# akloetgen/PARA-suite

Measured on AMD Instinct MI355X. Metric: aligned reads/sec (10Mx50bp PAR-CLIP vs hg19-size genome) on MI355X; SAM bit-exact vs own CPU restatement (parity unpinned), higher is better.
Workload: dtype u64

## Files before the change

para-suite_amd/capi.py:

```python
import ctypes as C
import os

import numpy as np

_HERE = os.path.dirname(os.path.abspath(__file__))
SO_PATH = os.environ.get("PARASUITE_LIB") or os.path.join(_HERE, "libparasuite_hip.so")


class IndexInfo(C.Structure):
    _fields_ = [("seq_len", C.c_uint64), ("l_pac", C.c_uint64), ("primary", C.c_uint64), ("L2", C.c_uint64 * 5),
                ("n_blocks", C.c_uint64), ("n_sa", C.c_uint64), ("device_bytes", C.c_uint64),
                ("n_contigs", C.c_int32), ("n_holes", C.c_int32), ("sa_rounds", C.c_int32), ("sa_intv", C.c_int32),
                ("build_ms", C.c_double), ("jump_levels", C.c_int32), ("pad_", C.c_int32)]


class Timing(C.Structure):
    _fields_ = [("ms_width", C.c_double), ("ms_backtrack", C.c_double), ("ms_compact", C.c_double),
                ("ms_select", C.c_double), ("ms_sa2pos", C.c_double), ("ms_refine", C.c_double),
                ("ms_host_post", C.c_double), ("ms_total", C.c_double), ("n_width_launches", C.c_int32),
                ("n_backtrack_launches", C.c_int32), ("n_overflow_tier1", C.c_int64), ("n_overflow_tier2", C.c_int64),
                ("ms_classify", C.c_double), ("ms_rows", C.c_double), ("ms_sel_hard", C.c_double), ("ms_sel_easy", C.c_double),
                ("bt_begin_ms", C.c_double), ("bt_end_ms", C.c_double)]


# ... 192 lines not shown
        k = np.ascontiguousarray(keys, dtype=np.uint8)
        out = np.empty(k.size, dtype=np.int32)
        _chk(lib().ps_ctx_order_sort(self.h, k.ctypes.data, k.size, out.ctypes.data))
        return out

    def export_blob(self, which, dev_ptr, nbytes):
        _chk(lib().ps_ctx_export_blob(self.h, which, dev_ptr, nbytes))

    def bwt_syms_chunked(self, chunk_blocks=1 << 20):
        info = self.info()
        blk = self.fetch(0).view("<u4").reshape(-1, 16)
        out = np.empty(blk.shape[0] * 192, dtype=np.uint8)
        sh = np.arange(32, dtype=np.uint32)[None, None, :]
        for a in range(0, blk.shape[0], chunk_blocks):
            lo = (blk[a:a + chunk_blocks, 4:10, None] >> sh) & 1
            hi = (blk[a:a + chunk_blocks, 10:16, None] >> sh) & 1
            out[a * 192:(a + lo.shape[0]) * 192] = (lo | (hi << 1)).astype(np.uint8).reshape(-1)
        return out[:info.seq_len]

    def bwt_syms(self):
        blk = self.fetch(0).view("<u4").reshape(-1, 16)
        return self.bwt_syms_chunked(), blk[:, :4]

    RI_WORDS = 20

    def read_iters(self):
        n = lib().ps_ctx_read_iters(self.h, None, 0)
        out = np.zeros(n, dtype=np.uint32)
        lib().ps_ctx_read_iters(self.h, out.ctypes.data, n)
        return out

    def batch_from_fastq(self, path):
        return Batch(lib().ps_batch_from_fastq(self.h, path.encode()), self)

    def batch_from_codes(self, codes):
        c = np.ascontiguousarray(codes, dtype=np.uint8)
        return Batch(lib().ps_batch_from_codes(self.h, c.shape[0], c.shape[1], c.ctypes.data), self)


class Batch:
    def __init__(self, handle, ctx):
        if not handle:
            raise PsError(lib().ps_last_error().decode())
        self.h = handle
        self.ctx = ctx

    def free(self):
# ... 228 lines not shown
```

para-suite_amd/csrc/ps_effort.hip:

```cpp
#include <hip/hip_runtime.h>
#include "ps_core.h"
#include <stdexcept>
#include "ps_kernels.h"
#include "ps_budget.h"

namespace ps {

struct EChain {
    bwtint k, l;
    uint32_t cost_lo, cost_hi;
    int piece;
    int n_rs;
    int cl_n, cl_last;
    uint32_t cl_lo, cl_hi;
};
__device__ __forceinline__ void echain_restart(const EffortArgs &a, EChain &c, bool lo_half)
{
    c.k = 0; c.l = a.ix.seq_len; c.piece = 0; c.cl_n = 0; ++c.n_rs;
    if (lo_half) c.cost_lo += (uint32_t)a.c_restart; else c.cost_hi += (uint32_t)a.c_restart;
}
__device__ __forceinline__ void echain_step(const EffortArgs &a, EChain &c, int sym, uint32_t cw, int pos, bool lo_half, LaneStats &st)
{
    uint32_t ck[4], cl[4];
    occ_pair4(a.ix.blocks, a.ix.primary, c.k, c.l, ck, cl, st);
    if (sym < 4) {
        const uint32_t ok = sel4(ck, sym), ol = sel4(cl, sym);
        if (ok < ol) { const bwtint b = L2_of(a.ix, sym); c.k = b + ok + 1; c.l = b + ol; ++c.piece; return; }
    }
    int best = -1; uint32_t best_cost = 0xffu;
    if (c.l - c.k < (bwtint)a.w_pin) {
#pragma unroll
        for (int t = 0; t < 4; ++t) {
            const uint32_t ct = (cw >> (8 * t)) & 0xffu;
            if (t != sym && ck[t] < cl[t] && ct < best_cost) { best = t; best_cost = ct; }
        }
    }
    if (best < 0) { echain_restart(a, c, lo_half); return; }
    const int d = pos > c.cl_last ? pos - c.cl_last : c.cl_last - pos;
    if (c.cl_n > 0 && d <= 4) ++c.cl_n; else { c.cl_n = 1; c.cl_lo = c.cost_lo; c.cl_hi = c.cost_hi; }
    c.cl_last = pos;
    if (lo_half) c.cost_lo += best_cost; else c.cost_hi += best_cost;
    if (c.cl_n >= 3) {
        c.k = 0; c.l = a.ix.seq_len; c.piece = 0; c.cl_n = 0; ++c.n_rs;
        return;
    }
    const bwtint b = L2_of(a.ix, best);
    c.k = b + sel4(ck, best) + 1; c.l = b + sel4(cl, best); ++c.piece;
}

__global__ void __launch_bounds__(256, 8) k_effort(EffortArgs a)
{
    const int lane = threadIdx.x & 63;
    const bool is_b = lane >= 32;
    const int wave = (int)((blockIdx.x * blockDim.x + threadIdx.x) >> 6), n_waves = (int)((gridDim.x * blockDim.x) >> 6);
    LaneStats st = {0, 0, 0, 0, 0, 0, 0, 0};
    for (int r = wave * 32 + (lane & 31); r < a.n_reads; r += n_waves * 32) {
        const int len = a.lens ? a.lens[r] : a.len, half = len >> 1;
        EChain C = {0, a.ix.seq_len, 0, 0, 0, 0, 0, 0, 0, 0};
        uint32_t bw = 0, mw = 0;
#pragma unroll 1
        for (int i = 0; i < len; ++i) {
            const int j = is_b ? i : len - 1 - i;
            if (i == 0 || (j & 15) == (is_b ? 0 : 15)) bw = a.bases[(size_t)(j >> 4) * a.n_reads + opaque_lane(r)];
            if (i == 0 || (j & 31) == (is_b ? 0 : 31)) mw = a.nmask[(size_t)(j >> 5) * a.n_reads + opaque_lane(r)];
            const int bs = ((mw >> (j & 31)) & 1u) ? 4 : (int)((bw >> (2 * (j & 15))) & 3u);
            const int sc = bs > 3 ? 4 : 3 - bs;
            const uint32_t cws = cost_word(a.s_pk, sc);
            const uint32_t cw = is_b ? cws : __builtin_bswap32(cws);
            echain_step(a, C, is_b ? sc : bs, cw, j, j < half, st);
        }
        const uint32_t mine = C.cost_lo + C.cost_hi;
        const uint32_t tb = (uint32_t)__shfl((int)mine, lane | 32, 64), ta = mine;
        const int b_rs = __shfl(C.n_rs, lane | 32, 64), a_rs = C.n_rs;
        if (!is_b) {
            const uint32_t e = a_rs == 0 ? (b_rs == 0 && tb < ta ? tb : ta) : (b_rs == 0 ? tb : (ta > tb ? ta : tb));
            a.est[r] = (uint8_t)(e > 255u ? 255u : e);
            if (a.est_ab) a.est_ab[r] = (uint16_t)((ta > 127u ? 127u : ta) | (a_rs ? 0x80u : 0u) | ((tb > 127u ? 127u : tb) << 8) | (b_rs ? 0x8000u : 0u));
        }
    }
}

template <int G>
__global__ void __launch_bounds__(256) k_effort_model(EffortModelArgs a)
{
    const int lane = threadIdx.x & 63, u = lane & (G - 1);
    const int per_wave = 64 / G;
    const long long wave = ((long long)blockIdx.x * blockDim.x + threadIdx.x) >> 6, n_waves = ((long long)gridDim.x * blockDim.x) >> 6;
    for (long long r0 = wave * per_wave + lane / G; r0 < a.n_reads; r0 += n_waves * per_wave) {
        const int r = (int)r0;
        const int len = a.lens ? a.lens[r] : a.len;
        const int own = (a.lens && a.units_by_len) ? (int)a.units_by_len[len] : a.max_units;
        int B = (int)a.est[r] + a.u_tight;
        if (B > own) B = own;
        float w = u == 0 ? 1.f : 0.f;
        float tot = 0.f, phi_rows = a.rows;
        const int depth = len < a.depth ? len : a.depth;
        const int rem = B - u;
        const int m = rem >= 0 ? (int)(((uint32_t)rem * a.inv_c_min) >> 16) : -1;
        const int srem = a.seed_units - u;
        const bool seed_ok = srem > 0 && (int)(((uint32_t)srem * a.inv_c_min) >> 16) >= 1;
// ... 76 lines not shown
```

para-suite_amd/csrc/ps_kernels.h:

```cpp
#pragma once
#include <hip/hip_runtime.h>
#include "ps_types.h"
#include "ps_budget.h"

namespace ps {

static const int PS_MAX_CIGAR = 16;

struct WidthArgs {
    IndexView ix;
    int n_reads, len, seed_len, use_seed;
    const int32_t *lens;
    const uint32_t *bases; const uint32_t *nmask;
    uint32_t *w; uint32_t *cwb; uint32_t *cswb;
    KStats *stats;
};

struct EffortArgs {
    IndexView ix;
    int n_reads, len;
    const int32_t *lens;
    const uint32_t *bases; const uint32_t *nmask;
    uint32_t s_pk[5];
    int c_restart;
    uint32_t w_pin;
    uint8_t *est;
    uint16_t *est_ab;
};

struct EffortModelArgs {
    int n_reads, len;
    const int32_t *lens; const uint8_t *units_by_len;
    const uint32_t *bases; const uint32_t *nmask; const uint32_t *cwb;
    const uint8_t *est;
    uint32_t s_pk[5]; uint32_t inv_c_min;
    int max_units, u_tight, seed_units, use_seed, seed_len;
    int max_gapo, indel_end_skip, u_gapo_ins, u_gapo_del;
    int depth;
    float rows;
    int log_scale;
    uint8_t *key; float *pred;
};

struct RefineItem { int32_t read; bwtint rb; int32_t ref_shift; int32_t strand; };
struct RefineArgs {
    IndexView ix;
    int n_items, len, n_reads;
    const int32_t *lens;
    const uint32_t *bases; const uint32_t *nmask;
    const RefineItem *items;
// ... 24 lines not shown
```

para-suite_amd/csrc/ps_kernels.hip:

```cpp
#include <hip/hip_runtime.h>
#include <algorithm>
#include <cstdlib>
#include <stdexcept>
#include <string>
#include "ps_core.h"
#include "ps_narrow.h"
#include "ps_kernels.h"

namespace ps {

static const int PS_Q_CHUNK = 64;
#ifndef PS_BT_WAVES
#define PS_BT_WAVES 4
#endif

__device__ __forceinline__ unsigned long long wave_sum(unsigned long long v)
{
    for (int o = 32; o > 0; o >>= 1) v += __shfl_xor(v, o, 64);
    return v;
}
__device__ __forceinline__ void flush_stats(KStats *ks, const LaneStats &st)
{
    if (!ks) return;
    unsigned long long v[8] = {st.pairs, st.same, st.nodes, st.pushes, st.pops, st.lf, st.iters, st.exact};
// ... 207 lines not shown
                unsigned int at = atomicAdd(a.big_next, 1u) % n_big;
                for (int tries = 0; tries < 256; ++tries) {
                    if (atomicCAS(a.big_busy + at, 0u, 1u) == 0u) { slot = at; break; }
                    at = at + 1u == n_big ? 0u : at + 1u;
                }
            }
            slot = (unsigned int)__shfl((int)slot, src, 64);
            const unsigned int n_copy = (unsigned int)__shfl((int)nl_bump(L), src, 64);
            const unsigned long long from = (unsigned long long)__shfl((long long)reinterpret_cast<unsigned long long>(m.pool), src, 64);
            if (slot < n_big) {
                const uint4 *sp = reinterpret_cast<const uint4 *>(from);
                uint4 *dp = reinterpret_cast<uint4 *>(a.big_pool + (size_t)slot * h.big_cap * sizeof(Entry16));
                for (unsigned int e = (unsigned int)lane; e < n_copy; e += 64u) dp[e] = sp[e];
                __threadfence();
                if (lane == src) { m.pool = dp; L.ctl = nl_set_mode(L.ctl | NL_BIG, M_EXPAND); }
            } else if (lane == src) L.ctl = nl_set_mode(nl_set_status(L.ctl, RS_OVERFLOW_POOL), M_POP);
        }
        nt_iter<STATS, NB32>(a, h, L, st, m, fetch_r, serve_hit, &clk);
        if (STATS && a.read_iters) {
            const int now = nl_mode(L.ctl);
            if (mode == M_FETCH && now != M_FETCH && now != M_EXIT) {
                iters0 = st.iters - 1u;
                const int len = nl_len(L), sl = h.seed_len();
                a.read_iters[PS_RI_WORDS * (size_t)L.r + 2] = (uint32_t)(m.cw[len - 1] & 0x7f) | ((h.use_seed() && sl > 0 && sl < len ? (uint32_t)(m.csw[sl - 1] & 0x7f) : 0u) << 8) | (a.est_ab ? (uint32_t)a.est_ab[L.r] << 16 : 0u);
                const uint32_t *cw32 = reinterpret_cast<const uint32_t *>(m.cw);
                for (int p = 0; p < 16; ++p) a.read_iters[PS_RI_WORDS * (size_t)L.r + 4 + p] = p < lm_ncw(len) ? cw32[p] : 0u;
            }
            if (mode != M_FETCH && mode != M_EXIT && now == M_FETCH) {
                uint32_t *ri = a.read_iters + PS_RI_WORDS * (size_t)L.r;
                ri[0] = st.iters - iters0; ri[1] = nl_bump(L);
                ri[3] = (uint32_t)nl_best_score(L) | ((uint32_t)nl_max_units(L) << 8) | ((uint32_t)nl_n_aln(L.ctl) << 16);
            }
        }
    }
    if (STATS) {
        if (lane == 0) st.lf = (uint32_t)((wall_clock64() - t_start) >> 4);
#ifdef PS_STAMPS
        st.nodes = lane == 0 ? (uint32_t)(clk.tm[0] >> 6) : 0; st.pushes = lane == 0 ? (uint32_t)(clk.tm[1] >> 6) : 0;
        st.pops = lane == 0 ? (uint32_t)(clk.tm[2] >> 6) : 0; st.exact = lane == 0 ? (uint32_t)(clk.tm[3] >> 6) : 0;
#endif
        flush_stats(a.stats, st);
    } else {
        st.nodes = st.pushes = st.pops = st.iters = st.exact = st.lf = 0;
        flush_stats(a.stats, st);
    }
}

__global__ void __launch_bounds__(256) k_sa2pos(IndexView ix, const bwtint *rows, bwtint *out, int n, KStats *stats)
{
    const int stride = gridDim.x * blockDim.x;
    int item = blockIdx.x * blockDim.x + threadIdx.x;
    LaneStats st = {0, 0, 0, 0, 0, 0, 0, 0};
    bool have = false; bwtint row = 0; uint32_t steps = 0;
    while (true) {
// ... 146 lines not shown
```

para-suite_amd/csrc/ps_narrow.h:

```cpp
#pragma once
#include "ps_core.h"

namespace ps {

PS_HD int nw_i(uint32_t wa) { return (int)(wa & 0xffu); }
PS_HD int nw_ldp(uint32_t wa) { return (int)((wa >> 8) & 0xffu); }
PS_HD int nw_mm(uint32_t wa) { return (int)((wa >> 16) & 0xffu); }
PS_HD int nw_state(uint32_t wa) { return (int)((wa >> 24) & 3u); }
PS_HD int nw_gapo(uint32_t wa) { return (int)((wa >> 26) & 7u); }
PS_HD int nw_gape(uint32_t wa) { return (int)(wa >> 29); }
PS_HD int nw_ins(uint32_t wb) { return (int)(wb & 7u); }
PS_HD int nw_del(uint32_t wb) { return (int)((wb >> 3) & 7u); }
PS_HD uint32_t nw_c(uint32_t wb) { return (wb >> 6) & 7u; }
PS_HD int nw_score(uint32_t wb) { return (int)((wb >> 9) & 0x7fu); }
static const uint32_t NW_KEEP = 0xFCFF0000u;
static const uint32_t NW_C_MASK = 7u << 6;
static const uint32_t NW_ROOT_C = 4u;

PS_HD int nl_mode(uint32_t ctl) { return (int)(ctl & 7u); }
PS_HD uint32_t nl_set_mode(uint32_t ctl, int mode) { return (ctl & ~7u) | (uint32_t)mode; }
static const uint32_t NL_HAVE_CUR = 8u, NL_STATUS = 7u << 4, NL_BIG = 1u << 7;
PS_HD int nl_status(uint32_t ctl) { return (int)((ctl >> 4) & 7u); }
PS_HD uint32_t nl_set_status(uint32_t ctl, int s) { return (ctl & ~NL_STATUS) | ((uint32_t)s << 4); }
PS_HD int nl_n_aln(uint32_t ctl) { return (int)(ctl >> 16); }

struct NLane {
    uint32_t kr, lr, wa, wb;
    uint32_t ctl;
    int r;
    uint32_t lim;
    uint32_t nsb;
    uint32_t n_phantom;
    uint32_t fh;
    uint32_t bm0, bm1;
    uint32_t rn0, rn1;
};
PS_HD int nl_best_score(const NLane &L) { return (int)(L.lim & 0xffu); }
PS_HD int nl_max_units(const NLane &L) { return (int)((L.lim >> 8) & 0xffu); }
PS_HD int nl_len(const NLane &L) { return (int)((L.lim >> 16) & 0xffu); }
PS_HD int nl_n_stack(const NLane &L) { return (int)(L.nsb & 0xffffu); }
PS_HD uint32_t nl_bump(const NLane &L) { return L.nsb >> 16; }
PS_HD uint32_t nl_phantom(const NLane &L) { return L.n_phantom & 0x00FFFFFFu; }
PS_HD int nl_est(const NLane &L) { return (int)(L.n_phantom >> 24); }

// ... 90 lines not shown
        empty = ps[2 * c] >= ps[2 * c + 1];
        kr = ps[2 * c] + 1u; lr = ps[2 * c + 1];
    }
    uint32_t ck[4] = {0, 0, 0, 0}, cl[4] = {0, 0, 0, 0};
    LaneStats st;
    if (!empty) nt_occ<false>(h, c, kr, lr, ck, cl, st);
    uint32_t *out = table + (size_t)(jump_level_off(d) + s) * PS_JUMP_SLOT_WORDS;
    for (int j = 0; j < 4; ++j) { out[2 * j] = ck[j]; out[2 * j + 1] = cl[j]; }
}

PS_HD int nt_seq_at(const BtMem &m, const NLane &L, int j, int len, int max_len)
{
    const int p = len - 1 - j;
    const uint32_t b = (m.rb[p >> 4] >> (2 * (p & 15))) & 3u;
    const uint32_t nw = lm_nmask_in_regs(max_len) ? (p < 32 ? L.rn0 : L.rn1) : m.rn[p >> 5];
    return ((nw >> (p & 31)) & 1u) ? 4 : 3 - (int)b;
}

PS_HD void nt_heads_init(BtMem &m, int n_buckets)
{
    uint32_t *hw = reinterpret_cast<uint32_t *>(m.heads16);
    for (int p = 0; p < (n_buckets + 1) >> 1; ++p) hw[p] = 0xFFFFFFFFu;
}
PS_COLD void nt_restart_without_estimate(const BtArgs &a, NLane &L, BtMem &m)
{
    L.ctl = (L.ctl & NL_BIG) | (uint32_t)M_POP | NL_HAVE_CUR;
    L.kr = 0; L.lr = (uint32_t)a.ix.seq_len; L.wa = (uint32_t)nl_len(L); L.wb = NW_ROOT_C << 6;
    L.lim = (L.lim & 0x00FFFF00u) | 0xffu;
    L.nsb = 0; L.bm0 = L.bm1 = 0; L.fh = 0xffffu; L.n_phantom = 0xFF000000u;
    nt_heads_init(m, a.md.n_buckets);
}
PS_HD void nt_finish_read(const BtArgs &a, NLane &L)
{
    a.n_aln[L.r] = nl_n_aln(L.ctl);
    a.status[L.r] = (uint8_t)nl_status(L.ctl);
    L.ctl = nl_set_mode(L.ctl, M_FETCH);
}

PS_COLD void nt_hit(const BtArgs &a, NLane &L, BtMem &m)
{
    const Model &md = a.md;
    const uint32_t c = nw_c(L.wb);
    if (a.ix.jump && c != NW_ROOT_C) {
        const int d = nt_depth(nl_len(L), L.wa, L.wb);
        if (d < a.ix.jump_levels) {
            const uint32_t *ps = a.ix.jump + (size_t)(jump_level_off(d - 1) + (L.kr >> 2)) * PS_JUMP_SLOT_WORDS;
            L.kr = ps[2 * c] + 1u; L.lr = ps[2 * c + 1];
        }
    }
    const bwtint base = c == NW_ROOT_C ? (a.ix.seq_len & ~(bwtint)0xFFFFFFFFull) : a.ix.L2[c];
    const bwtint k = base + L.kr, l = base + L.lr;
    const int score = nw_score(L.wb), n_gapo = nw_gapo(L.wa);
    const int units = md.profile ? score : nw_mm(L.wa) + n_gapo + (md.mode_gape ? nw_gape(L.wa) : 0);
    const int n_aln = nl_n_aln(L.ctl);
    if (n_aln == 0) {
        if (units > nl_est(L)) { nt_restart_without_estimate(a, L, m); return; }
        int t = units + md.u_tight;
        const int own = nl_max_units(L);
        t = t > own ? own : t;
        L.lim = (L.lim & 0x00FF0000u) | (uint32_t)score | ((uint32_t)t << 8);
    }
    if (score == nl_best_score(L)) {
        const unsigned long long s = (unsigned long long)(L.lim >> 24) + (unsigned long long)(l - k) + 1ull;
        L.lim = (L.lim & 0x00FFFFFFu) | ((s > 255ull ? 255u : (uint32_t)s) << 24);
    } else if ((int)(L.lim >> 24) > md.max_top2) { nt_finish_read(a, L); return; }
    AlnRec *out = a.alns + (size_t)L.r * a.aln_cap;
    if (n_gapo) {
        for (int j = 0; j < n_aln; ++j)
            if (out[j].k == k && out[j].l == l) return;
    }
    {
        const uint32_t shadow = a.ix.seq_len > 0xFFFFFFFFull ? 0xFFFFFFFFu : (uint32_t)a.ix.seq_len;
        uint32_t x = (uint32_t)(l - k + 1), j = 0, prev = 0;
        const int lim = nw_ldp(L.wa);
        for (int i = 0; i < lim; ++i) {
            size_t off = (size_t)i * a.n_reads + L.r;
            uint32_t w = a.w[off];
            int bid = m.cw[i] & 0x7f;
            if (w > x) { w -= x; a.w[off] = w; }
// ... 102 lines not shown
PS_HD int nt_head(const BtArgs &a, const BtHot &h, NLane &L, LaneStats &st, BtMem &m, int fetch_r, bool serve_hit)
{
    int mode = nl_mode(L.ctl);
    if (mode == M_EXIT || mode == M_GROW) return 0;
    if (STATS) ++st.iters;
    if (mode == M_HIT) {
        if (!serve_hit) return 0;
        L.ctl = nl_set_mode(L.ctl, M_POP);
        { NLane t = L; nt_hit(a, t, m); L = t; }
        return 0;
    }
    if (mode == M_FETCH) {
        if (fetch_r < 0) return 0;
        if (fetch_r >= (int)h.n_reads) { L.ctl = nl_set_mode(L.ctl, M_EXIT); return 0; }
        { NLane t = L; const bool ok = nt_fetch(a, t, m, fetch_r); L = t; if (!ok) return 0; }
        L.ctl = nl_set_mode(L.ctl, M_POP);
        mode = M_POP;
    }
    if (mode == M_POP) {
        const int n_virtual = nl_n_stack(L) + ((L.ctl & NL_HAVE_CUR) ? 1 : 0);
        if (nl_phantom(L) && (long long)n_virtual + (long long)nl_phantom(L) > (long long)h.max_entries) {
            L.ctl = nl_set_status(L.ctl, RS_OVERFLOW_POOL); nt_finish_read(a, L); return 0;
        }
        if (n_virtual == 0 && nl_est(L) != 255 && nl_n_aln(L.ctl) == 0 && nl_status(L.ctl) == RS_OK) { NLane t = L; nt_restart_without_estimate(a, t, m); L = t; return 0; }
        if (n_virtual == 0 || n_virtual > (int)h.max_entries || nl_status(L.ctl) != RS_OK) { nt_finish_read(a, L); return 0; }
        if (L.ctl & NL_HAVE_CUR) L.ctl &= ~NL_HAVE_CUR;
        else { nt_pop<NB32>(L, m); if (STATS) ++st.pops; }
        L.ctl = nl_set_mode(L.ctl, M_POP);
        const int score = nw_score(L.wb), i1 = nw_i(L.wa);
        if (score > nl_best_score(L) + h.s_stop()) { nt_finish_read(a, L); return 0; }
        const int rem = nl_max_units(L) - nt_units(h, L.wa, L.wb);
        if (rem < 0) return 0;
        const int mleft = (int)(ps_mul24((uint32_t)rem, h.inv_c_min) >> 16);
        if (i1 > 0 && mleft < (int)(m.cw[i1 - 1] & 0x7f)) return 0;
        if (i1 == 0) { L.ctl = nl_set_mode(L.ctl, M_HIT); return 0; }
        const int st_ = nw_state(L.wa);
        mode = (mleft == 0 && (st_ == ST_M || h.mode_gape() || nw_gape(L.wa) == h.max_gape())) ? M_EXACT : M_EXPAND;
    }
    return mode;
}

struct NtStep { uint32_t ck[4], cl[4]; uint32_t cw_i, cw_im1, cs_i, cs_im1; int s, i; bool in_seed, tm, ctm; };

template <bool STATS>
PS_HD void nt_step_occ(const BtHot &h, NLane &L, LaneStats &st, BtMem &m, NtStep &q)
{
    const int len = nl_len(L), max_len = h.len();
    const int i = nw_i(L.wa) - 1;
    q.i = i;
    q.cw_i = m.cw[i]; q.cw_im1 = m.cw[i > 0 ? i - 1 : 0];
    const int ii = i - (len - h.seed_len());
    q.in_seed = h.use_seed() && len > h.seed_len() && ii > 0;
    q.cs_i = q.in_seed ? m.csw[ii] : 0u; q.cs_im1 = q.in_seed ? m.csw[ii - 1] : 0u;
    q.s = nt_seq_at(m, L, i, len, max_len);
    const int depth = nt_depth(len, L.wa, L.wb);
    q.tm = depth < (int)h.jump_levels; q.ctm = depth + 1 < (int)h.jump_levels;
    if (!q.tm) nt_occ<STATS>(h, nw_c(L.wb), L.kr, L.lr, q.ck, q.cl, st);
    else nt_jump(h, depth, L.kr, q.ck, q.cl);
// ... 33 lines not shown
    const int m_seed = srem <= 0 ? 0 : (int)(ps_mul24((uint32_t)srem, inv) >> 16);
    bool allow_diff = true, allow_M = true;
    const int bnd_same = i > 0 ? (int)(cw_im1 & 0x7f) : 0;
    const int bnd_del = (int)(cw_i & 0x7f);
    if (i > 0) {
        if (bnd_same > mleft - 1) allow_diff = false;
        else if (bnd_same == mleft - 1 && bnd_del == mleft - 1 && (cw_i & 0x80u)) allow_M = false;
        if (in_seed) {
            const int s1 = (int)(cs_im1 & 0x7f), s0 = (int)(cs_i & 0x7f);
            if (s1 > m_seed - 1) allow_diff = false;
            else if (s1 == m_seed - 1 && s0 == m_seed - 1 && (cs_i & 0x80u)) allow_M = false;
        }
    }
    const int e_go = nw_gapo(L.wa), e_ge = nw_gape(L.wa), e_st = nw_state(L.wa);
    const int tmp = e_go + e_ge;
    const bool gap_ok = allow_diff && i >= h.indel_end_skip() + tmp && len - i >= h.indel_end_skip() + tmp;
    const bool from_m = e_st == ST_M, from_i = e_st == ST_I, from_d = e_st == ST_D;
    const uint32_t wa_keep = L.wa & NW_KEEP, pos2 = (uint32_t)i | ((uint32_t)i << 8);
    const uint32_t wb0 = L.wb & 0x1ffu;
    const uint32_t pkr = L.kr, plr = L.lr;
    const int need_same = (int)ps_mul24((uint32_t)bnd_same, h.c_min), need_del = (int)ps_mul24((uint32_t)bnd_del, h.c_min);
    const int cap_rem = nl_est(L) - e_sc, ut = h.u_tight();
    const int cap_same = cap_rem + (ut > need_same ? ut - need_same : 0), cap_del = cap_rem + (ut > need_del ? ut - need_del : 0);
    const int thr_same = (rem - need_same) < cap_same ? (rem - need_same) : cap_same, thr_del = (rem - need_del) < cap_del ? (rem - need_del) : cap_del;
    uint32_t phantom = 0, gmask = 0;
    int sc[9];
    uint32_t wa_i, wa_d;
    {
        const bool open = from_m && e_go < h.max_gapo(), ext = from_i && e_ge < h.max_gape();
        const int c = open ? h.u_gapo_ins() : h.u_gape();
        sc[0] = e_sc + (open ? h.s_gapo_ins() : h.s_gape());
        const bool cand = gap_ok && (open || ext) && c <= rem, go = cand && c <= thr_same;
        gmask |= go ? 1u : 0u;
        phantom += (cand && !go) ? 1u : 0u;
        wa_i = wa_keep + pos2 + ((uint32_t)ST_I << 24) + (open ? 1u << 26 : 1u << 29);
    }
    {
        const uint32_t occ = tm ? plr : plr - pkr + 1u;
        const bool open = from_m && e_go < h.max_gapo();
        const bool ext = from_d && e_ge < h.max_gape() && ((e_ge + e_go) * h.u_tight() < max_units || occ < (uint32_t)h.max_del_occ());
        const int c = open ? h.u_gapo_del() : h.u_gape();
        const int scd = e_sc + (open ? h.s_gapo_del() : h.s_gape());
        const bool cand = gap_ok && (open || ext) && c <= rem, go = cand && c <= thr_del;
        const uint32_t ne = (ck[0] < cl[0] ? 2u : 0u) | (ck[1] < cl[1] ? 4u : 0u) | (ck[2] < cl[2] ? 8u : 0u) | (ck[3] < cl[3] ? 16u : 0u);
        gmask |= go ? ne : 0u;
        if (cand && !go) phantom += ps_popc(ne);
        sc[1] = sc[2] = sc[3] = sc[4] = scd;
        wa_d = wa_keep + ((uint32_t)(i + 1) | ((uint32_t)(i + 1) << 8)) + ((uint32_t)ST_D << 24) + (open ? 1u << 26 : 1u << 29);
    }
    const bool do_mm = allow_diff && allow_M;
    const uint32_t s_word = cost_word(h.s_pk, s), u_word = h.profile() ? s_word : cost_word(h.u_pk, s);
    uint32_t xk[4], xl[4];
#pragma unroll
    for (int j = 1; j <= 4; ++j) {
        const int c = (s + j) & 3;
        xk[j - 1] = sel4(ck, c); xl[j - 1] = sel4(cl, c);
        sc[4 + j] = 0;
        if (j < 4 || s > 3) {
            const int cu = (int)((u_word >> (8 * c)) & 0xffu);
            sc[4 + j] = e_sc + (int)((s_word >> (8 * c)) & 0xffu);
            const bool cand = do_mm && xk[j - 1] < xl[j - 1] && cu <= rem, go = cand && cu <= thr_same;
            gmask |= go ? 1u << (4 + j) : 0u;
            phantom += (cand && !go) ? 1u : 0u;
        }
    }
    const uint32_t n_push = ps_popc(gmask), fr = L.fh;
    const bool reuse = fr != 0xffffu && n_push != 0u;
    const uint32_t slot0 = (L.nsb >> 16) - (reuse ? 1u : 0u);
    L.nsb += n_push + ((n_push - (reuse ? 1u : 0u)) << 16);
    L.fh = n_push ? 0xffffu : fr;
    if (STATS) st.pushes += n_push;
    uint32_t idx[9], raw[9];
#pragma unroll
    for (int j = 0; j < 9; ++j) {
        idx[j] = 0; raw[j] = 0;
        if ((gmask >> j) & 1u) {
            const uint32_t rank = ps_popc(gmask & ((1u << j) - 1u));
            idx[j] = (reuse && rank == 0u) ? fr : slot0 + rank;
            raw[j] = m.heads16[sc[j]];
            m.heads16[sc[j]] = (uint16_t)idx[j];
            if (NB32 || sc[j] < 32) L.bm0 |= 1u << sc[j]; else L.bm1 |= 1u << (sc[j] - 32);
        }
    }
#ifdef __HIP_DEVICE_COMPILE__
    asm volatile("" : "+v"(raw[0]), "+v"(raw[1]), "+v"(raw[2]), "+v"(raw[3]), "+v"(raw[4]), "+v"(raw[5]), "+v"(raw[6]), "+v"(raw[7]), "+v"(raw[8]));
#endif
// ... 1 lines not shown
#define NT_NEXT(j) (raw[j] << 16)
    if (gmask & 1u) { Entry16 e; e.k = pkr; e.l = plr; e.a = wa_i; e.b = (wb0 + 1u) | ((uint32_t)sc[0] << 9) | NT_NEXT(0); store16(pool + idx[0], e); }
    {
        const uint32_t wb_d = ((wb0 & 0x3fu) + (1u << 3)) | ((uint32_t)sc[1] << 9);
#pragma unroll
        for (int c = 0; c < 4; ++c)
            if ((gmask >> (1 + c)) & 1u) { Entry16 e; e.k = ctm ? (pkr << 2) | (uint32_t)c : ck[c] + 1u; e.l = ctm ? cl[c] - ck[c] : cl[c]; e.a = wa_d; e.b = wb_d | ((uint32_t)c << 6) | NT_NEXT(1 + c); store16(pool + idx[1 + c], e); }
    }
    {
        const uint32_t wa_x = wa_keep + pos2 + (1u << 16), wb_x = wb0 & 0x3fu;
#pragma unroll
        for (int j = 1; j <= 4; ++j) {
            const uint32_t c = (uint32_t)((s + j) & 3);
            if ((gmask >> (4 + j)) & 1u) { Entry16 e; e.k = ctm ? (pkr << 2) | c : xk[j - 1] + 1u; e.l = ctm ? xl[j - 1] - xk[j - 1] : xl[j - 1]; e.a = wa_x; e.b = wb_x | (c << 6) | ((uint32_t)sc[4 + j] << 9) | NT_NEXT(4 + j); store16(pool + idx[4 + j], e); }
        }
    }
#undef NT_NEXT
    L.ctl = nl_set_mode(L.ctl, M_POP);
    if (s < 4 && xk[3] < xl[3]) {
        L.kr = ctm ? (pkr << 2) | (uint32_t)s : xk[3] + 1u; L.lr = ctm ? xl[3] - xk[3] : xl[3]; L.wa = wa_keep + (uint32_t)i; L.wb = (L.wb & ~NW_C_MASK) | ((uint32_t)s << 6);
        L.ctl |= NL_HAVE_CUR;
    }
    L.n_phantom += phantom;
}

template <bool STATS, bool NB32>
PS_HD void nt_iter(const BtArgs &a, const BtHot &h, NLane &L, LaneStats &st, BtMem &m, int fetch_r, bool serve_hit, NtClock *clk = nullptr)
{
    PS_USTAMP(clk, 0);
    const int mode = nt_head<STATS, NB32>(a, h, L, st, m, fetch_r, serve_hit);
    PS_USTAMP(clk, 1);
    NtStep q;
    if (mode) nt_step_occ<STATS>(h, L, st, m, q);
#if defined(PS_STAMPS) && defined(__HIP_DEVICE_COMPILE__)
    if (STATS && clk && mode) asm volatile("" :: "v"(q.ck[0]), "v"(q.cl[0]), "v"(q.ck[3]), "v"(q.cl[3]));
#endif
    PS_USTAMP(clk, 2);
    if (mode) nt_tail<STATS, NB32>(h, L, st, m, q, mode);
    PS_USTAMP(clk, 3);
}

}
```

para-suite_amd/csrc/ps_pipeline.hip:

```cpp
#include <hip/hip_runtime.h>
#include <mutex>
#include <optional>
#include <hipcub/hipcub.hpp>
#include <algorithm>
#include <atomic>
#include <chrono>
#include <cmath>
#include <cstdio>
#include <cstring>
#include <functional>
#include <thread>
#include "ps_pipeline.h"
#include "ps_par.h"
#include "ps_core.h"

namespace ps {

typedef std::chrono::steady_clock Clock;
static double ms_since(Clock::time_point t0) { return std::chrono::duration<double, std::milli>(Clock::now() - t0).count(); }

void require_device(int device)
{
    int n = 0;
    hipError_t e = hipGetDeviceCount(&n);
// ... 261 lines not shown
    explicit EvTimer(hipStream_t st) : s(st) { PS_HIP(hipEventCreate(&a)); PS_HIP(hipEventCreate(&b)); PS_HIP(hipEventRecord(a, s)); }
    double stop() { mark(); return read(); }
    void mark() { PS_HIP(hipEventRecord(b, s)); }
    double read() { PS_HIP(hipEventSynchronize(b)); float ms = 0; PS_HIP(hipEventElapsedTime(&ms, a, b)); return ms; }
    void span(hipEvent_t ref, double &t_begin, double &t_end) { float x = 0, y = 0; if (ref && hipEventElapsedTime(&x, ref, a) == hipSuccess && hipEventElapsedTime(&y, ref, b) == hipSuccess) { t_begin = x; t_end = y; } }
    ~EvTimer() { (void)hipEventDestroy(a); (void)hipEventDestroy(b); }
};


static void run_search(Batch &b, const Model &md, int n, const uint32_t *d_bases, const uint32_t *d_nmask, const int32_t *d_lens,
                       uint32_t pool_cap, int aln_cap, AlnRec *alns, int32_t *n_aln, uint8_t *status, bool first_tier = false)
{
    Ctx *ctx = b.ctx; Work *wk = b.wk; hipStream_t s = wk->stream;
    const int len = md.len, seed_len = md.seed_len;
    uint32_t *w = wk->ws_get<uint32_t>("w", (size_t)(len + 1) * n);
    uint32_t *cwb = wk->ws_get<uint32_t>("cwb", (size_t)lm_ncw(len) * n);
    uint32_t *cswb = wk->ws_get<uint32_t>("cswb", (size_t)(lm_ncsw(seed_len) + 1) * n);
    WidthArgs wa;
    wa.ix = ctx->ix.view; wa.n_reads = n; wa.len = len; wa.lens = d_lens; wa.seed_len = seed_len; wa.use_seed = md.use_seed;
    wa.bases = d_bases; wa.nmask = d_nmask; wa.w = w; wa.cwb = cwb; wa.cswb = cswb; wa.stats = b.d_stats.p + 0;
    std::optional<EvTimer> t_width, t_order;
    t_width.emplace(s); launch_width(wa, s); PS_HIP(hipGetLastError()); t_width->mark(); ++b.tm.n_width_launches;
    const bool wide = launch_is_wide(md, pool_cap);
    const int32_t *d_order = nullptr; const uint8_t *d_est = nullptr; const uint16_t *d_est_ab = nullptr;
    if (!wide) {
        const char *eo = std::getenv("PS_ORDER");
        const int mode = eo ? std::atoi(eo) : 1;
        int min_n = 4096;
        if (const char *e = std::getenv("PS_ORDER_MIN")) min_n = std::max(1, std::atoi(e));
        if (mode > 0 && n >= min_n && md.max_units >= md.c_min) {
            t_order.emplace(s);
            uint8_t *est = wk->ws_get<uint8_t>("est", (size_t)n), *key = wk->ws_get<uint8_t>("okey", (size_t)n);
            int32_t *order = wk->ws_get<int32_t>("order", (size_t)n);
            EffortArgs ea;
            ea.ix = ctx->ix.view; ea.n_reads = n; ea.len = len; ea.lens = d_lens; ea.bases = d_bases; ea.nmask = d_nmask; ea.est = est;
            int csum = 0;
            for (int c = 0; c < 5; ++c) ea.s_pk[c] = md.u_mm_pk[c];
            for (int sc = 0; sc < 4; ++sc) for (int tc = 0; tc < 4; ++tc) if (sc != tc) csum += md.u_mm[sc][tc];
            ea.c_restart = std::max(1, (csum + 6) / 12);
            if (const char *e = std::getenv("PS_ORDER_RESTART")) ea.c_restart = std::max(1, std::atoi(e));
            ea.w_pin = 16;
            if (const char *e = std::getenv("PS_ORDER_WPIN")) ea.w_pin = (uint32_t)std::max(1, std::atoi(e));
            int lv = 0; while (lv < 31 && (ctx->ix.view.seq_len >> (2 * lv)) > 0) ++lv;
            ea.est_ab = ctx->want_read_iters ? wk->ws_get<uint16_t>("est_ab", (size_t)n) : nullptr;
            launch_effort(ea, s);
            d_est_ab = ea.est_ab;
            if (mode == 2) {
                int cap = 255;
                if (const char *e = std::getenv("PS_ORDER_CAP")) cap = std::max(1, std::min(255, std::atoi(e)));
                hipLaunchKernelGGL(k_order_keys, dim3(std::min((n + 255) / 256, 4096)), dim3(256), 0, s, est, n, cap, key);
            } else {
                EffortModelArgs em;
                em.n_reads = n; em.len = len; em.lens = d_lens; em.units_by_len = nullptr; em.bases = d_bases; em.nmask = d_nmask; em.cwb = cwb; em.est = est;
                for (int c = 0; c < 5; ++c) em.s_pk[c] = md.u_mm_pk[c];
                em.inv_c_min = (uint32_t)md.inv_c_min; em.max_units = md.max_units; em.u_tight = md.u_tight;
                em.seed_units = md.max_seed_diff * md.u_tight; em.use_seed = md.use_seed; em.seed_len = md.seed_len;
                em.max_gapo = md.max_gapo; em.indel_end_skip = md.indel_end_skip; em.u_gapo_ins = md.u_gapo_ins; em.u_gapo_del = md.u_gapo_del;
                em.depth = lv + 3; em.rows = (float)ctx->ix.view.seq_len; em.log_scale = 8;
                if (const char *e = std::getenv("PS_ORDER_SCALE")) em.log_scale = std::max(1, std::min(12, std::atoi(e)));
                if (d_lens) {
                    uint8_t *tab = wk->pin_get<uint8_t>("units_by_len_h2", 256);
                    for (int l2 = 0; l2 < 256; ++l2) { const int u = budget_diffs(ctx->opt, l2) * (ctx->opt.profile ? ctx->opt.unit : 1); tab[l2] = (uint8_t)(u > 255 ? 255 : u); }
                    uint8_t *d_tab = wk->ws_get<uint8_t>("units_by_len2", 256);
                    PS_HIP(hipMemcpyAsync(d_tab, tab, 256, hipMemcpyHostToDevice, s));
                    em.units_by_len = d_tab;
                }
                em.key = key; em.pred = nullptr;
                launch_effort_model(em, s);
            }
            launch_order_sort(key, n, wk->ws_get<uint32_t>("order_tmp", order_sort_tmp_words(n)), order, s);
            PS_HIP(hipGetLastError());
            t_order->mark();
            d_order = order; d_est = est;
        }
    }
    int dev_cus = 256;
    { hipDeviceProp_t p; if (hipGetDeviceProperties(&p, ctx->device) == hipSuccess && p.multiProcessorCount > 0) dev_cus = p.multiProcessorCount; }
    const int lm = lm_bytes(len, seed_len, md.n_buckets, wide);
    int per_cu = (int)((size_t)(160 * 1024) / ((size_t)256 * lm));
    if (per_cu < 1) throw Error("read length / score range too large for the per-lane LDS state");
    { const char *e = std::getenv("PS_MAX_PER_CU"); const int cap = e ? std::atoi(e) : 4; if (per_cu > cap) per_cu = cap; }
    int blocks = ctx->bt_blocks > 0 ? ctx->bt_blocks : dev_cus * per_cu;
    int need = (n + 255) / 256;
    if (blocks > need) blocks = need;
    const size_t per_lane = (size_t)pool_cap * (wide ? sizeof(Entry) : 16) + (wide ? PS_MAX_BUCKETS * 4 : 0);
    const size_t max_lanes = ((size_t)(wide ? 32 : 64) << 30) / per_lane;
    if ((size_t)blocks * 256 > max_lanes) blocks = (int)std::max<size_t>(1, max_lanes / 256);
    const int n_lanes = blocks * 256;
    uint8_t *pool = wk->ws_get<uint8_t>("pool", (size_t)n_lanes * pool_cap * (wide ? sizeof(Entry) : 16));
    uint32_t *heads = wide ? wk->ws_get<uint32_t>("heads", (size_t)n_lanes * PS_MAX_BUCKETS) : nullptr;
    uint32_t *queue = wk->ws_get<uint32_t>("queue", 16);
    PS_HIP(hipMemsetAsync(queue, 0, 64, s));
    BtArgs a; std::memset(&a, 0, sizeof a);
    a.ix = ctx->ix.view; a.md = md; a.n_reads = n; a.len = len; a.lens = d_lens; a.n_lanes = n_lanes;
    if (d_lens) {
        uint8_t *tab = wk->pin_get<uint8_t>("units_by_len_h", 256);
// ... 707 lines not shown
```

para-suite_amd/csrc/ps_types.h:

```cpp
#pragma once
#include <stdint.h>
#include <stddef.h>

#ifdef __HIPCC__
#define PS_HD __host__ __device__ __forceinline__
#define PS_COLD __host__ __device__ inline __attribute__((noinline))
#else
#define PS_HD inline
#define PS_COLD inline
#endif

namespace ps {

typedef uint64_t bwtint;
static const bwtint PS_MAX_ROWS = (1ull << 33) - 64;

static const int PS_BLK_SYMS = 192;
struct OccBlock { uint32_t cnt[4]; uint32_t sym[12]; };

struct IndexView {
    const OccBlock *blocks;
    const uint32_t *sa;
    const uint32_t *sa_hi;
    const uint8_t  *pac;
// ... 20 lines not shown

struct Entry {
    bwtint k, l;
    uint16_t score, units;
    uint8_t i, last_diff_pos, n_mm, n_gapo, n_gape, n_ins, n_del, state;
    uint32_t next;
};
static const uint32_t PS_NIL = 0xFFFFFFFFu;
enum { ST_M = 0, ST_I = 1, ST_D = 2 };

struct AlnRec {
    bwtint k, l;
    uint16_t score, units;
    uint8_t n_mm, n_gapo, n_gape, n_ins, n_del, pad[7];
};

enum { RS_OK = 0, RS_OVERFLOW_POOL = 1, RS_OVERFLOW_ALN = 2, RS_BAD_SCORE = 3,
       RS_OVERFLOW_DEEP = 4 };

struct KStats {
    unsigned long long occ_pairs, occ_same_blk, nodes, pushes, pops, lf_steps, iters, exact_steps;
};

static const int PS_RI_WORDS = 20;
struct BtArgs {
    IndexView ix;
    Model md;
    int n_reads, len, n_lanes;
    const int32_t *lens;
    const uint8_t *units_by_len;
    const uint32_t *bases; const uint32_t *nmask; int n_bw, n_mw;
    uint32_t *w; const uint32_t *cwb; const uint32_t *cswb;
    AlnRec *alns; int aln_cap; int32_t *n_aln; uint8_t *status;
    void *pool; uint32_t pool_cap;
    uint32_t *heads;
    int wide;
    uint8_t *big_pool; uint32_t big_cap, n_big; uint32_t *big_busy; uint32_t *big_next;
    uint32_t *queue;
    const int32_t *order;
    const uint8_t *est; const uint16_t *est_ab;
    int cap_est;
    uint32_t *read_iters;
    int hit_min;
    int fetch_min;
    KStats *stats;
};

}
```

Before: 8.972 million.

## Tighten effort-estimate cap and restart only when search was actually capped

```diff
diff --git a/para-suite_amd/capi.py b/para-suite_amd/capi.py
--- a/para-suite_amd/capi.py
+++ b/para-suite_amd/capi.py
@@ -238,7 +238,7 @@
         blk = self.fetch(0).view("<u4").reshape(-1, 16)
         return self.bwt_syms_chunked(), blk[:, :4]
 
-    RI_WORDS = 20
+    RI_WORDS = 21
 
     def read_iters(self):
         n = lib().ps_ctx_read_iters(self.h, None, 0)
diff --git a/para-suite_amd/csrc/ps_effort.hip b/para-suite_amd/csrc/ps_effort.hip
--- a/para-suite_amd/csrc/ps_effort.hip
+++ b/para-suite_amd/csrc/ps_effort.hip
@@ -14,9 +14,10 @@
     int cl_n, cl_last;
     uint32_t cl_lo, cl_hi;
 };
+static const int ECH_RS = 1, ECH_RS_LO = 2, ECH_RS_HI = 4;
 __device__ __forceinline__ void echain_restart(const EffortArgs &a, EChain &c, bool lo_half)
 {
-    c.k = 0; c.l = a.ix.seq_len; c.piece = 0; c.cl_n = 0; ++c.n_rs;
+    c.k = 0; c.l = a.ix.seq_len; c.piece = 0; c.cl_n = 0; c.n_rs |= ECH_RS | (lo_half ? ECH_RS_LO : ECH_RS_HI);
     if (lo_half) c.cost_lo += (uint32_t)a.c_restart; else c.cost_hi += (uint32_t)a.c_restart;
 }
 __device__ __forceinline__ void echain_step(const EffortArgs &a, EChain &c, int sym, uint32_t cw, int pos, bool lo_half, LaneStats &st)
@@ -41,7 +42,7 @@
     c.cl_last = pos;
     if (lo_half) c.cost_lo += best_cost; else c.cost_hi += best_cost;
     if (c.cl_n >= 3) {
-        c.k = 0; c.l = a.ix.seq_len; c.piece = 0; c.cl_n = 0; ++c.n_rs;
+        c.k = 0; c.l = a.ix.seq_len; c.piece = 0; c.cl_n = 0; c.n_rs |= ECH_RS | (lo_half ? ECH_RS_LO : ECH_RS_HI);
         return;
     }
     const bwtint b = L2_of(a.ix, best);
@@ -72,10 +73,15 @@
         const uint32_t mine = C.cost_lo + C.cost_hi;
         const uint32_t tb = (uint32_t)__shfl((int)mine, lane | 32, 64), ta = mine;
         const int b_rs = __shfl(C.n_rs, lane | 32, 64), a_rs = C.n_rs;
+        const uint32_t b_hi = (uint32_t)__shfl((int)C.cost_hi, lane | 32, 64), a_lo = C.cost_lo;
         if (!is_b) {
             const uint32_t e = a_rs == 0 ? (b_rs == 0 && tb < ta ? tb : ta) : (b_rs == 0 ? tb : (ta > tb ? ta : tb));
             a.est[r] = (uint8_t)(e > 255u ? 255u : e);
-            if (a.est_ab) a.est_ab[r] = (uint16_t)((ta > 127u ? 127u : ta) | (a_rs ? 0x80u : 0u) | ((tb > 127u ? 127u : tb) << 8) | (b_rs ? 0x8000u : 0u));
+            uint32_t c = e;
+            if (a.cap_rule && a_rs && b_rs && !(a_rs & ECH_RS_LO) && !(b_rs & ECH_RS_HI)) c = a_lo + b_hi;
+            a.cap[r] = (uint8_t)(c > 255u ? 255u : c);
+            if (a.est_ab) a.est_ab[r] = (ta > 127u ? 127u : ta) | (a_rs ? 0x80u : 0u) | ((tb > 127u ? 127u : tb) << 8) | (b_rs ? 0x8000u : 0u) |
+                                        ((a_lo > 127u ? 127u : a_lo) << 16) | ((a_rs & ECH_RS_LO) ? 0x800000u : 0u) | ((b_hi > 127u ? 127u : b_hi) << 24) | ((b_rs & ECH_RS_HI) ? 0x80000000u : 0u);
         }
     }
 }
diff --git a/para-suite_amd/csrc/ps_kernels.h b/para-suite_amd/csrc/ps_kernels.h
--- a/para-suite_amd/csrc/ps_kernels.h
+++ b/para-suite_amd/csrc/ps_kernels.h
@@ -25,7 +25,9 @@
     int c_restart;
     uint32_t w_pin;
     uint8_t *est;
-    uint16_t *est_ab;
+    uint8_t *cap;
+    int cap_rule;
+    uint32_t *est_ab;
 };
 
 struct EffortModelArgs {
diff --git a/para-suite_amd/csrc/ps_kernels.hip b/para-suite_amd/csrc/ps_kernels.hip
--- a/para-suite_amd/csrc/ps_kernels.hip
+++ b/para-suite_amd/csrc/ps_kernels.hip
@@ -253,7 +253,8 @@
             if (mode == M_FETCH && now != M_FETCH && now != M_EXIT) {
                 iters0 = st.iters - 1u;
                 const int len = nl_len(L), sl = h.seed_len();
-                a.read_iters[PS_RI_WORDS * (size_t)L.r + 2] = (uint32_t)(m.cw[len - 1] & 0x7f) | ((h.use_seed() && sl > 0 && sl < len ? (uint32_t)(m.csw[sl - 1] & 0x7f) : 0u) << 8) | (a.est_ab ? (uint32_t)a.est_ab[L.r] << 16 : 0u);
+                a.read_iters[PS_RI_WORDS * (size_t)L.r + 2] = (uint32_t)(m.cw[len - 1] & 0x7f) | ((h.use_seed() && sl > 0 && sl < len ? (uint32_t)(m.csw[sl - 1] & 0x7f) : 0u) << 8) | (a.est_ab ? (a.est_ab[L.r] & 0xffffu) << 16 : 0u);
+                a.read_iters[PS_RI_WORDS * (size_t)L.r + 20] = a.est_ab ? a.est_ab[L.r] >> 16 : 0u;
                 const uint32_t *cw32 = reinterpret_cast<const uint32_t *>(m.cw);
                 for (int p = 0; p < 16; ++p) a.read_iters[PS_RI_WORDS * (size_t)L.r + 4 + p] = p < lm_ncw(len) ? cw32[p] : 0u;
             }
@@ -261,6 +262,7 @@
                 uint32_t *ri = a.read_iters + PS_RI_WORDS * (size_t)L.r;
                 ri[0] = st.iters - iters0; ri[1] = nl_bump(L);
                 ri[3] = (uint32_t)nl_best_score(L) | ((uint32_t)nl_max_units(L) << 8) | ((uint32_t)nl_n_aln(L.ctl) << 16);
+                ri[20] |= (L.ctl & NL_RESTARTED) ? 1u << 16 : 0u;
             }
         }
     }
diff --git a/para-suite_amd/csrc/ps_narrow.h b/para-suite_amd/csrc/ps_narrow.h
--- a/para-suite_amd/csrc/ps_narrow.h
+++ b/para-suite_amd/csrc/ps_narrow.h
@@ -20,6 +20,8 @@
 PS_HD int nl_mode(uint32_t ctl) { return (int)(ctl & 7u); }
 PS_HD uint32_t nl_set_mode(uint32_t ctl, int mode) { return (ctl & ~7u) | (uint32_t)mode; }
 static const uint32_t NL_HAVE_CUR = 8u, NL_STATUS = 7u << 4, NL_BIG = 1u << 7;
+static const uint32_t NL_RESTARTED = 1u << 9;
+static const uint32_t NL_CAPPED = 1u << 8;
 PS_HD int nl_status(uint32_t ctl) { return (int)((ctl >> 4) & 7u); }
 PS_HD uint32_t nl_set_status(uint32_t ctl, int s) { return (ctl & ~NL_STATUS) | ((uint32_t)s << 4); }
 PS_HD int nl_n_aln(uint32_t ctl) { return (int)(ctl >> 16); }
@@ -156,14 +158,15 @@
     uint32_t *hw = reinterpret_cast<uint32_t *>(m.heads16);
     for (int p = 0; p < (n_buckets + 1) >> 1; ++p) hw[p] = 0xFFFFFFFFu;
 }
-PS_COLD void nt_restart_without_estimate(const BtArgs &a, NLane &L, BtMem &m)
-{
-    L.ctl = (L.ctl & NL_BIG) | (uint32_t)M_POP | NL_HAVE_CUR;
+PS_COLD void nt_restart_read(const BtArgs &a, NLane &L, BtMem &m, int est)
+{
+    L.ctl = (L.ctl & NL_BIG) | NL_RESTARTED | (uint32_t)M_POP | NL_HAVE_CUR;
     L.kr = 0; L.lr = (uint32_t)a.ix.seq_len; L.wa = (uint32_t)nl_len(L); L.wb = NW_ROOT_C << 6;
     L.lim = (L.lim & 0x00FFFF00u) | 0xffu;
-    L.nsb = 0; L.bm0 = L.bm1 = 0; L.fh = 0xffffu; L.n_phantom = 0xFF000000u;
+    L.nsb = 0; L.bm0 = L.bm1 = 0; L.fh = 0xffffu; L.n_phantom = (uint32_t)est << 24;
     nt_heads_init(m, a.md.n_buckets);
 }
+PS_HD void nt_restart_without_estimate(const BtArgs &a, NLane &L, BtMem &m) { nt_restart_read(a, L, m, 255); }
 PS_HD void nt_finish_read(const BtArgs &a, NLane &L)
 {
     a.n_aln[L.r] = nl_n_aln(L.ctl);
@@ -188,7 +191,10 @@
     const int units = md.profile ? score : nw_mm(L.wa) + n_gapo + (md.mode_gape ? nw_gape(L.wa) : 0);
     const int n_aln = nl_n_aln(L.ctl);
     if (n_aln == 0) {
-        if (units > nl_est(L)) { nt_restart_without_estimate(a, L, m); return; }
+        if (units > nl_est(L)) {
+            if (L.ctl & NL_CAPPED) { nt_restart_read(a, L, m, units + md.u_tight < nl_max_units(L) ? units : 255); return; }
+            L.n_phantom |= 0xFF000000u;
+        }
         int t = units + md.u_tight;
         const int own = nl_max_units(L);
         t = t > own ? own : t;
@@ -337,7 +343,7 @@
         if (nl_phantom(L) && (long long)n_virtual + (long long)nl_phantom(L) > (long long)h.max_entries) {
             L.ctl = nl_set_status(L.ctl, RS_OVERFLOW_POOL); nt_finish_read(a, L); return 0;
         }
-        if (n_virtual == 0 && nl_est(L) != 255 && nl_n_aln(L.ctl) == 0 && nl_status(L.ctl) == RS_OK) { NLane t = L; nt_restart_without_estimate(a, t, m); L = t; return 0; }
+        if (n_virtual == 0 && (L.ctl & NL_CAPPED) && nl_n_aln(L.ctl) == 0 && nl_status(L.ctl) == RS_OK) { NLane t = L; nt_restart_without_estimate(a, t, m); L = t; return 0; }
         if (n_virtual == 0 || n_virtual > (int)h.max_entries || nl_status(L.ctl) != RS_OK) { nt_finish_read(a, L); return 0; }
         if (L.ctl & NL_HAVE_CUR) L.ctl &= ~NL_HAVE_CUR;
         else { nt_pop<NB32>(L, m); if (STATS) ++st.pops; }
@@ -349,6 +355,7 @@
         const int mleft = (int)(ps_mul24((uint32_t)rem, h.inv_c_min) >> 16);
         if (i1 > 0 && mleft < (int)(m.cw[i1 - 1] & 0x7f)) return 0;
         if (i1 == 0) { L.ctl = nl_set_mode(L.ctl, M_HIT); return 0; }
+        if (score > nl_est(L) && (L.ctl & NL_CAPPED) && nl_n_aln(L.ctl) == 0) { NLane t = L; nt_restart_without_estimate(a, t, m); L = t; return 0; }
         const int st_ = nw_state(L.wa);
         mode = (mleft == 0 && (st_ == ST_M || h.mode_gape() || nw_gape(L.wa) == h.max_gape())) ? M_EXACT : M_EXPAND;
     }
@@ -428,8 +435,10 @@
     const int need_same = (int)ps_mul24((uint32_t)bnd_same, h.c_min), need_del = (int)ps_mul24((uint32_t)bnd_del, h.c_min);
     const int cap_rem = nl_est(L) - e_sc, ut = h.u_tight();
     const int cap_same = cap_rem + (ut > need_same ? ut - need_same : 0), cap_del = cap_rem + (ut > need_del ? ut - need_del : 0);
-    const int thr_same = (rem - need_same) < cap_same ? (rem - need_same) : cap_same, thr_del = (rem - need_del) < cap_del ? (rem - need_del) : cap_del;
+    const int own_same = rem - need_same, own_del = rem - need_del;
+    const int thr_same = own_same < cap_same ? own_same : cap_same, thr_del = own_del < cap_del ? own_del : cap_del;
     uint32_t phantom = 0, gmask = 0;
+    bool capped = false;
     int sc[9];
     uint32_t wa_i, wa_d;
     {
@@ -439,6 +448,7 @@
         const bool cand = gap_ok && (open || ext) && c <= rem, go = cand && c <= thr_same;
         gmask |= go ? 1u : 0u;
         phantom += (cand && !go) ? 1u : 0u;
+        capped |= cand && !go && c <= own_same;
         wa_i = wa_keep + pos2 + ((uint32_t)ST_I << 24) + (open ? 1u << 26 : 1u << 29);
     }
     {
@@ -451,6 +461,7 @@
         const uint32_t ne = (ck[0] < cl[0] ? 2u : 0u) | (ck[1] < cl[1] ? 4u : 0u) | (ck[2] < cl[2] ? 8u : 0u) | (ck[3] < cl[3] ? 16u : 0u);
         gmask |= go ? ne : 0u;
         if (cand && !go) phantom += ps_popc(ne);
+        capped |= cand && !go && ne != 0u && c <= own_del;
         sc[1] = sc[2] = sc[3] = sc[4] = scd;
         wa_d = wa_keep + ((uint32_t)(i + 1) | ((uint32_t)(i + 1) << 8)) + ((uint32_t)ST_D << 24) + (open ? 1u << 26 : 1u << 29);
     }
@@ -468,6 +479,7 @@
             const bool cand = do_mm && xk[j - 1] < xl[j - 1] && cu <= rem, go = cand && cu <= thr_same;
             gmask |= go ? 1u << (4 + j) : 0u;
             phantom += (cand && !go) ? 1u : 0u;
+            capped |= cand && !go && cu <= own_same;
         }
     }
     const uint32_t n_push = ps_popc(gmask), fr = L.fh;
@@ -515,6 +527,7 @@
         L.ctl |= NL_HAVE_CUR;
     }
     L.n_phantom += phantom;
+    L.ctl |= capped ? NL_CAPPED : 0u;
 }
 
 template <bool STATS, bool NB32>
diff --git a/para-suite_amd/csrc/ps_pipeline.hip b/para-suite_amd/csrc/ps_pipeline.hip
--- a/para-suite_amd/csrc/ps_pipeline.hip
+++ b/para-suite_amd/csrc/ps_pipeline.hip
@@ -307,7 +307,7 @@
     std::optional<EvTimer> t_width, t_order;
     t_width.emplace(s); launch_width(wa, s); PS_HIP(hipGetLastError()); t_width->mark(); ++b.tm.n_width_launches;
     const bool wide = launch_is_wide(md, pool_cap);
-    const int32_t *d_order = nullptr; const uint8_t *d_est = nullptr; const uint16_t *d_est_ab = nullptr;
+    const int32_t *d_order = nullptr; const uint8_t *d_est = nullptr; const uint32_t *d_est_ab = nullptr;
     if (!wide) {
         const char *eo = std::getenv("PS_ORDER");
         const int mode = eo ? std::atoi(eo) : 1;
@@ -315,10 +315,12 @@
         if (const char *e = std::getenv("PS_ORDER_MIN")) min_n = std::max(1, std::atoi(e));
         if (mode > 0 && n >= min_n && md.max_units >= md.c_min) {
             t_order.emplace(s);
-            uint8_t *est = wk->ws_get<uint8_t>("est", (size_t)n), *key = wk->ws_get<uint8_t>("okey", (size_t)n);
+            uint8_t *est = wk->ws_get<uint8_t>("est", (size_t)n), *cap = wk->ws_get<uint8_t>("est_cap", (size_t)n), *key = wk->ws_get<uint8_t>("okey", (size_t)n);
             int32_t *order = wk->ws_get<int32_t>("order", (size_t)n);
             EffortArgs ea;
-            ea.ix = ctx->ix.view; ea.n_reads = n; ea.len = len; ea.lens = d_lens; ea.bases = d_bases; ea.nmask = d_nmask; ea.est = est;
+            ea.ix = ctx->ix.view; ea.n_reads = n; ea.len = len; ea.lens = d_lens; ea.bases = d_bases; ea.nmask = d_nmask; ea.est = est; ea.cap = cap;
+            ea.cap_rule = 1;
+            if (const char *e = std::getenv("PS_CAP_RULE")) ea.cap_rule = std::atoi(e) != 0 ? 1 : 0;
             int csum = 0;
             for (int c = 0; c < 5; ++c) ea.s_pk[c] = md.u_mm_pk[c];
             for (int sc = 0; sc < 4; ++sc) for (int tc = 0; tc < 4; ++tc) if (sc != tc) csum += md.u_mm[sc][tc];
@@ -327,7 +329,7 @@
             ea.w_pin = 16;
             if (const char *e = std::getenv("PS_ORDER_WPIN")) ea.w_pin = (uint32_t)std::max(1, std::atoi(e));
             int lv = 0; while (lv < 31 && (ctx->ix.view.seq_len >> (2 * lv)) > 0) ++lv;
-            ea.est_ab = ctx->want_read_iters ? wk->ws_get<uint16_t>("est_ab", (size_t)n) : nullptr;
+            ea.est_ab = ctx->want_read_iters ? wk->ws_get<uint32_t>("est_ab", (size_t)n) : nullptr;
             launch_effort(ea, s);
             d_est_ab = ea.est_ab;
             if (mode == 2) {
@@ -356,7 +358,7 @@
             launch_order_sort(key, n, wk->ws_get<uint32_t>("order_tmp", order_sort_tmp_words(n)), order, s);
             PS_HIP(hipGetLastError());
             t_order->mark();
-            d_order = order; d_est = est;
+            d_order = order; d_est = cap;
         }
     }
     int dev_cus = 256;
diff --git a/para-suite_amd/csrc/ps_types.h b/para-suite_amd/csrc/ps_types.h
--- a/para-suite_amd/csrc/ps_types.h
+++ b/para-suite_amd/csrc/ps_types.h
@@ -66,7 +66,7 @@
     unsigned long long occ_pairs, occ_same_blk, nodes, pushes, pops, lf_steps, iters, exact_steps;
 };
 
-static const int PS_RI_WORDS = 20;
+static const int PS_RI_WORDS = 21;
 struct BtArgs {
     IndexView ix;
     Model md;
@@ -82,7 +82,7 @@
     uint8_t *big_pool; uint32_t big_cap, n_big; uint32_t *big_busy; uint32_t *big_next;
     uint32_t *queue;
     const int32_t *order;
-    const uint8_t *est; const uint16_t *est_ab;
+    const uint8_t *est; const uint32_t *est_ab;
     int cap_est;
     uint32_t *read_iters;
     int hit_min;
```

Result: no change. 8.975 million, median of 3 (+0.0%).
